# facebookresearch/AudioDec

Measured on NVIDIA H100. Metric: 48 kHz audio samples/s, encode+quantize+lookup+decode (% HBM roofline in `roofline`), higher is better.
Workload: dtype f32

## Files before the change

audiodec_b200/csrc/wg_conv.cuh:

```cuda
#pragma once
#include <cuda_bf16.h>
#include <cuda_fp16.h>

#include "kernels.cuh"

namespace adec {

constexpr int TC_TT = 128;
constexpr int TC_CP = 32;
constexpr int TC_MIDP = 128;
constexpr float F16_LO_SCALE = 2048.f;
enum { PREC_BF16 = 1, PREC_TF32 = 2, PREC_F16 = 3 };

__device__ __forceinline__ void fence_async_smem() { asm volatile("fence.proxy.async.shared::cta;" ::: "memory"); }
__device__ __forceinline__ float tf32_rna(float x) {
    uint32_t r;
    asm("cvt.rna.tf32.f32 %0, %1;" : "=r"(r) : "f"(x));
    return __uint_as_float(r);
}

__device__ __forceinline__ uint64_t wg_desc(uint32_t saddr, uint32_t lbo_bytes) {
    return (uint64_t)((saddr & 0x3FFFF) >> 4) | ((uint64_t)((lbo_bytes >> 4) & 0x3FFF) << 16) | ((uint64_t)(128 >> 4) << 32);
}
__device__ __forceinline__ void wg_fence() { asm volatile("wgmma.fence.sync.aligned;" ::: "memory"); }
__device__ __forceinline__ void wg_commit() { asm volatile("wgmma.commit_group.sync.aligned;" ::: "memory"); }
__device__ __forceinline__ void wg_wait0() { asm volatile("wgmma.wait_group.sync.aligned 0;" ::: "memory"); }
template <int N>
__device__ __forceinline__ void wg_fence_regs(float (&d)[N]) {
#pragma unroll
    for (int i = 0; i < N; ++i) asm volatile("" : "+f"(d[i])::"memory");
}

template <int N, int PREC> struct Wgmma;
#define ADEC_WG_N32(PREC, TYPE, TAIL)                                                                                              \
    template <> struct Wgmma<32, PREC> {                                                                                           \
        __device__ __forceinline__ static void mma(float (&d)[16], uint64_t da, uint64_t db, uint32_t acc) {                     \
            asm volatile("{\n .reg .pred p;\n setp.ne.b32 p, %18, 0;\n wgmma.mma_async.sync.aligned.m64n32" TYPE                \
                         " {%0,%1,%2,%3,%4,%5,%6,%7,%8,%9,%10,%11,%12,%13,%14,%15}, %16, %17, p, 1, 1" TAIL ";\n}"                  \
                         : "+f"(d[0]), "+f"(d[1]), "+f"(d[2]), "+f"(d[3]), "+f"(d[4]), "+f"(d[5]), "+f"(d[6]), "+f"(d[7]),          \
                           "+f"(d[8]), "+f"(d[9]), "+f"(d[10]), "+f"(d[11]), "+f"(d[12]), "+f"(d[13]), "+f"(d[14]), "+f"(d[15])     \
                         : "l"(da), "l"(db), "r"(acc));                                                                            \
        }                                                                                                                          \
    };
#define ADEC_WG_N64(PREC, TYPE, TAIL)                                                                                              \
    template <> struct Wgmma<64, PREC> {                                                                                           \
        __device__ __forceinline__ static void mma(float (&d)[32], uint64_t da, uint64_t db, uint32_t acc) {                     \
            asm volatile("{\n .reg .pred p;\n setp.ne.b32 p, %34, 0;\n wgmma.mma_async.sync.aligned.m64n64" TYPE                \
                         " {%0,%1,%2,%3,%4,%5,%6,%7,%8,%9,%10,%11,%12,%13,%14,%15,%16,%17,%18,%19,%20,%21,%22,%23,%24,%25,%26,%27," \
                         "%28,%29,%30,%31}, %32, %33, p, 1, 1" TAIL ";\n}"                                                          \
                         : "+f"(d[0]), "+f"(d[1]), "+f"(d[2]), "+f"(d[3]), "+f"(d[4]), "+f"(d[5]), "+f"(d[6]), "+f"(d[7]),          \
                           "+f"(d[8]), "+f"(d[9]), "+f"(d[10]), "+f"(d[11]), "+f"(d[12]), "+f"(d[13]), "+f"(d[14]), "+f"(d[15]),    \
                           "+f"(d[16]), "+f"(d[17]), "+f"(d[18]), "+f"(d[19]), "+f"(d[20]), "+f"(d[21]), "+f"(d[22]), "+f"(d[23]),  \
                           "+f"(d[24]), "+f"(d[25]), "+f"(d[26]), "+f"(d[27]), "+f"(d[28]), "+f"(d[29]), "+f"(d[30]), "+f"(d[31])   \
                         : "l"(da), "l"(db), "r"(acc));                                                                            \
        }                                                                                                                          \
    };
ADEC_WG_N32(PREC_F16, "k16.f32.f16.f16", ", 0, 0")
ADEC_WG_N32(PREC_BF16, "k16.f32.bf16.bf16", ", 0, 0")
ADEC_WG_N32(PREC_TF32, "k8.f32.tf32.tf32", "")
ADEC_WG_N64(PREC_F16, "k16.f32.f16.f16", ", 0, 0")
ADEC_WG_N64(PREC_BF16, "k16.f32.bf16.bf16", ", 0, 0")
ADEC_WG_N64(PREC_TF32, "k8.f32.tf32.tf32", "")
#undef ADEC_WG_N32
#undef ADEC_WG_N64

template <int NT, int PREC> struct WgCfg {
    static constexpr int EB = PREC == PREC_TF32 ? 4 : 2;
    static constexpr int KBB = TC_CP * EB / 16;
    static constexpr int NPR = PREC == PREC_F16 ? 3 : PREC == PREC_TF32 ? 2 : 1;
    static constexpr int NPL = PREC == PREC_BF16 ? 1 : 2;
    static constexpr int TPG = PREC == PREC_TF32 ? 1 : 2;
    static constexpr int TAP_BYTES = NPR * KBB * NT * 16;
    static constexpr int STAGE_BYTES = TPG * TAP_BYTES;
    static constexpr int MID_BYTES = NPL * (NT * EB / 16) * TC_MIDP * 16;
    __host__ __device__ static constexpr int stages(bool fuse) { return PREC == PREC_TF32 && NT == 128 && fuse ? 1 : NT == 128 ? 2 : 3; }
    static constexpr int PW = NT < 64 ? NT : 64;
    static constexpr int NPROD = 96;
    static constexpr int THREADS = 256 + NPROD + 32;
    __host__ __device__ static constexpr int win_pitch(int wrows) { return ((wrows + 1) & ~3) + 2; }
    __host__ __device__ static constexpr int win_bytes(int wrows) { return NPL * KBB * win_pitch(wrows) * 16; }
    static int n_wbuf(int wrows, bool fuse) {
        const long long avail = 227 * 1024 - 512 - (long long)stages(fuse) * STAGE_BYTES - (fuse ? (long long)MID_BYTES : 0);
        const long long n = avail / win_bytes(wrows);
        return (int)(n > 4 ? 4 : n);
    }
    static size_t smem_bytes(int wrows, bool fuse) {
        return 512 + (size_t)stages(fuse) * STAGE_BYTES + (size_t)n_wbuf(wrows, fuse) * win_bytes(wrows) + (fuse ? (size_t)MID_BYTES : 0);
    }
};

template <int ACT>
__device__ __forceinline__ float4 apply_act_t(float4 v, float slope) {
    if (ACT == ACT_ELU) { v.x = act_elu(v.x); v.y = act_elu(v.y); v.z = act_elu(v.z); v.w = act_elu(v.w); }
    if (ACT == ACT_LRELU) { v.x = act_lrelu(v.x, slope); v.y = act_lrelu(v.y, slope); v.z = act_lrelu(v.z, slope); v.w = act_lrelu(v.w, slope); }
    return v;
}

__device__ __forceinline__ uint32_t h2_bits(__half2 h) { return *reinterpret_cast<const uint32_t*>(&h); }
__device__ __forceinline__ uint32_t b2_bits(__nv_bfloat162 h) { return *reinterpret_cast<const uint32_t*>(&h); }
template <int PREC>
__device__ __forceinline__ void split2(float x, float y, uint2& hi, uint2& lo) {
    if (PREC == PREC_F16) {
        const __half2 h = __floats2half2_rn(x, y);
        const float2 f = __half22float2(h);
        hi.x = h2_bits(h);
        lo.x = h2_bits(__floats2half2_rn((x - f.x) * F16_LO_SCALE, (y - f.y) * F16_LO_SCALE));
    } else if (PREC == PREC_TF32) {
        const float hx = tf32_rna(x), hy = tf32_rna(y);
        hi = make_uint2(__float_as_uint(hx), __float_as_uint(hy));
        lo = make_uint2(__float_as_uint(x - hx), __float_as_uint(y - hy));
    } else {
        hi.x = b2_bits(__floats2bfloat162_rn(x, y));
    }
}
template <int PREC>
__device__ __forceinline__ void split_store(unsigned char* hi, unsigned char* lo, size_t bstride, const float4 u, const float4 v) {
    uint2 h0, l0, h1, l1, h2, l2, h3, l3;
    split2<PREC>(u.x, u.y, h0, l0); split2<PREC>(u.z, u.w, h1, l1);
    split2<PREC>(v.x, v.y, h2, l2); split2<PREC>(v.z, v.w, h3, l3);
    if (PREC == PREC_TF32) {
        *reinterpret_cast<uint4*>(hi) = make_uint4(h0.x, h0.y, h1.x, h1.y);
        *reinterpret_cast<uint4*>(hi + bstride) = make_uint4(h2.x, h2.y, h3.x, h3.y);
        *reinterpret_cast<uint4*>(lo) = make_uint4(l0.x, l0.y, l1.x, l1.y);
        *reinterpret_cast<uint4*>(lo + bstride) = make_uint4(l2.x, l2.y, l3.x, l3.y);
    } else {
        *reinterpret_cast<uint4*>(hi) = make_uint4(h0.x, h1.x, h2.x, h3.x);
        if (PREC == PREC_F16) *reinterpret_cast<uint4*>(lo) = make_uint4(l0.x, l1.x, l2.x, l3.x);
    }
}

struct TileIter {
    int tile, xt, y, b, sx, sy, sb, nx, ny;
    __device__ __forceinline__ TileIter(int first, int step, int n_x, int n_y) {
        nx = n_x; ny = n_y; tile = first;
        xt = first % n_x;
        const int q = first / n_x;
        y = q % n_y; b = q / n_y;
        sx = step % n_x;
        const int sq = step / n_x;
        sy = sq % n_y; sb = sq / n_y;
    }
    __device__ __forceinline__ void next(int step) {
        tile += step;
        xt += sx;
        const int cx = xt >= nx ? 1 : 0;
        xt -= cx ? nx : 0;
        y += sy + cx;
        const int cy = y >= ny ? 1 : 0;
        y -= cy ? ny : 0;
        b += sb + cy;
    }
};

__device__ __forceinline__ float4 norm4(float4 x, const float* mean, const float* scale) {
    const float4 mu = *reinterpret_cast<const float4*>(mean);
    const float4 sc = *reinterpret_cast<const float4*>(scale);
    x.x = __fdiv_rn(x.x - mu.x, sc.x); x.y = __fdiv_rn(x.y - mu.y, sc.y);
    x.z = __fdiv_rn(x.z - mu.z, sc.z); x.w = __fdiv_rn(x.w - mu.w, sc.w);
    return x;
}

template <int NT, int PREC>
__device__ __forceinline__ void wg_group(float (&d)[WgCfg<NT, PREC>::PW / 2], uint32_t a_hi, uint32_t a_lo, uint32_t lbo, uint32_t tap_step,
                                         int ntaps, uint32_t bw) {
    using Cfg = WgCfg<NT, PREC>;
    constexpr int NKS = Cfg::KBB / 2, TPG = Cfg::TPG;
    constexpr uint32_t B_LBO = NT * 16u, B_KS = 2u * NT * 16u, B_T = Cfg::TAP_BYTES, B_PL = Cfg::KBB * NT * 16u;
    constexpr uint32_t PL_SMALL = PREC == PREC_F16 ? 2u : 0u;
    uint32_t acc = 0u;
    wg_fence_regs(d);
    wg_fence();
    if (PREC != PREC_BF16) {
#pragma unroll
        for (int t = 0; t < TPG; ++t)
#pragma unroll
            for (int ks = 0; ks < NKS; ++ks)
                if (t < ntaps) {
                    Wgmma<Cfg::PW, PREC>::mma(d, wg_desc(a_lo + t * tap_step + ks * 2u * lbo, lbo), wg_desc(bw + t * B_T + PL_SMALL * B_PL + ks * B_KS, B_LBO), acc);
                    acc = 1u;
                }
#pragma unroll
        for (int t = 0; t < TPG; ++t)
#pragma unroll
            for (int ks = 0; ks < NKS; ++ks)
                if (t < ntaps) Wgmma<Cfg::PW, PREC>::mma(d, wg_desc(a_hi + t * tap_step + ks * 2u * lbo, lbo), wg_desc(bw + t * B_T + B_PL + ks * B_KS, B_LBO), 1u);
    }
#pragma unroll
    for (int t = 0; t < TPG; ++t)
#pragma unroll
        for (int ks = 0; ks < NKS; ++ks)
            if (t < ntaps) {
                Wgmma<Cfg::PW, PREC>::mma(d, wg_desc(a_hi + t * tap_step + ks * 2u * lbo, lbo), wg_desc(bw + t * B_T + ks * B_KS, B_LBO), acc);
                acc = 1u;
            }
    wg_commit();
    wg_wait0();
    wg_fence_regs(d);
}

template <int NT, bool FUSE, int PRE, int PREC>
__global__ void __launch_bounds__(WgCfg<NT, PREC>::THREADS, 1) wg_conv_kernel(const ConvArgs a, int n_xtiles, int n_ytiles, int n_tiles) {
    using Cfg = WgCfg<NT, PREC>;
    constexpr int S = Cfg::stages(FUSE), CP = TC_CP, TT = TC_TT, KBB = Cfg::KBB, EB = Cfg::EB, TPG = Cfg::TPG, PW = Cfg::PW;
    constexpr int NPROD = Cfg::NPROD, WWARP = (256 + NPROD) / 32;
    constexpr int STAGE_BYTES = Cfg::STAGE_BYTES, TAP_BYTES = Cfg::TAP_BYTES;
    constexpr int NH = NT / PW;
    constexpr int NACC = NT / 2;
    constexpr int MBLK = NT * EB / 16;

    extern __shared__ __align__(128) unsigned char smem_raw[];
    uint64_t* b_full = reinterpret_cast<uint64_t*>(smem_raw);
    uint64_t* b_empty = b_full + S;
    uint64_t* w_full = b_empty + S;
    uint64_t* w_empty = w_full + 4;
    unsigned char* bst = smem_raw + 512;
    const int wrows = TT + (a.Ktaps - 1) * a.dil;
    const int wrp = Cfg::win_pitch(wrows);
    const int win_b = Cfg::win_bytes(wrows);
    unsigned char* wbuf0 = bst + S * STAGE_BYTES;
    unsigned char* mbuf = wbuf0 + (size_t)a.n_wbuf * win_b;

    const int tid = threadIdx.x, lane = tid & 31;
    const int warp = __shfl_sync(0xffffffffu, tid >> 5, 0);
    unsigned long long kt0 = 0;
    long long kc0 = 0;
    if (a.dbg && blockIdx.x == 0 && tid == 0) { asm volatile("mov.u64 %0, %%globaltimer;" : "=l"(kt0)); kc0 = clock64(); }
    if (tid == 0) {
        for (int s = 0; s < S; ++s) { mbar_init(&b_full[s], 1); mbar_init(&b_empty[s], 2); }
        for (int i = 0; i < 4; ++i) { mbar_init(&w_full[i], NPROD); mbar_init(&w_empty[i], 2); }
        mbar_fence_init();
    }
    __syncthreads();
    asm volatile("griddepcontrol.launch_dependents;" ::: "memory");
    if (warp != WWARP) asm volatile("griddepcontrol.wait;" ::: "memory");

    if (warp == WWARP) {
        if (lane == 0) {
            int c = 0;
            auto stream = [&](const unsigned char* base, int pieces, int taps) {
                for (int p = 0; p < pieces; ++p)
                    for (int t0 = 0; t0 < taps; t0 += TPG, ++c) {
                        const int s = c % S, it = c / S;
                        const uint32_t bytes = (uint32_t)(taps - t0 >= TPG ? TPG : taps - t0) * TAP_BYTES;
                        if (it > 0) mbar_wait(&b_empty[s], (it - 1) & 1, 100);
                        mbar_arrive_expect_tx(&b_full[s], bytes);
                        bulk_g2s(bst + s * STAGE_BYTES, base + ((long long)p * taps + t0) * TAP_BYTES, bytes, &b_full[s]);
                    }
            };
            const unsigned char* w1 = reinterpret_cast<const unsigned char*>(a.w);
            const unsigned char* w2 = reinterpret_cast<const unsigned char*>(a.w2);
            for (TileIter it(blockIdx.x, gridDim.x, n_xtiles, n_ytiles); it.tile < n_tiles; it.next(gridDim.x)) {
                stream(w1 + (long long)it.y * a.w_tile_floats * 4, a.n_pieces, a.Ktaps);
                if (FUSE) stream(w2, NT / CP, 1);
            }
        }
    } else if (warp >= 8) {
        const int pt = tid - 256;
        int wb = 0, wround = 0;
        constexpr int RPP = NPROD / 4;
        constexpr int UNR = 6;
        constexpr int UNR_E = 6;
        const int c8 = pt & 3, m0 = pt >> 2;
        const size_t bstride = (size_t)wrp * 16;
        const bool halves = a.RG > 1 && a.Cin < 8;
        for (TileIter it(blockIdx.x, gridDim.x, n_xtiles, n_ytiles); it.tile < n_tiles; it.next(gridDim.x)) {
            const int xt = it.xt, y = it.y, b = it.b;
            int g = 0, co_tile = y;
            if (a.n_co_tiles != n_ytiles) { g = y / a.n_co_tiles; co_tile = y - g * a.n_co_tiles; }
            const int j0 = xt * TT;
            const float* xg = a.x + (long long)b * a.x_bs + g * a.x_goff;
            const float* sg = a.st_in + (long long)b * a.P * a.st_ld + g * a.st_goff;
            for (int p = 0; p < a.n_pieces; ++p) {
                const int buf = wb;
                const uint32_t wpar = (uint32_t)(wround - 1) & 1u;
                bool waited = wround == 0;
                if (++wb == a.n_wbuf) { wb = 0; ++wround; }
                unsigned char* hi = wbuf0 + (size_t)buf * win_b + (size_t)c8 * (KBB / 4) * bstride;
                unsigned char* lo = hi + (size_t)KBB * bstride;
                const int q = p * CP + c8 * 8;
                int r = 0, ci = q;
                if (a.RG > 1) { r = q >> a.lgCin; ci = q & (a.Cin - 1); }
                const long long i_first = (long long)j0 * a.RG + r;
                const long long i_last = (long long)(j0 + wrows - 1) * a.RG + r;
                if (i_first >= a.P && i_last - a.P < a.T && PRE != ACT_NORM && !halves && !a.stack_L) {
                    const float* xp = xg + ci + (i_first - a.P + (long long)m0 * a.RG) * a.ldx;
                    const long long xstep = (long long)RPP * a.RG * a.ldx;
                    for (int mb = m0; mb < wrows; mb += RPP * UNR, xp += xstep * UNR) {
                        float4 u[UNR], v[UNR];
#pragma unroll
                        for (int k = 0; k < UNR; ++k)
                            if (mb + k * RPP < wrows) {
                                u[k] = __ldg(reinterpret_cast<const float4*>(xp + k * xstep));
                                v[k] = __ldg(reinterpret_cast<const float4*>(xp + k * xstep) + 1);
                            }
                        if (!waited) { mbar_wait(&w_empty[buf], wpar, 500); waited = true; }
#pragma unroll
                        for (int k = 0; k < UNR; ++k) {
                            const int m = mb + k * RPP;
                            if (m < wrows) split_store<PREC>(hi + m * 16, lo + m * 16, bstride, apply_act_t<PRE>(u[k], a.slope), apply_act_t<PRE>(v[k], a.slope));
                        }
                    }
                } else {
                    int ci2 = ci + 4;
                    for (int mb = m0; mb < wrows; mb += RPP * UNR_E) {
                        float4 u[UNR_E], v[UNR_E];
                        unsigned act = 0u;
#pragma unroll
                        for (int k = 0; k < UNR_E; ++k) {
                            const int m = mb + k * RPP;
                            u[k] = v[k] = make_float4(0.f, 0.f, 0.f, 0.f);
                            if (m < wrows) {
                                int ml = j0 + m;
                                const float* xs = xg;
                                const float* ss = sg;
                                bool live = true;
                                if (a.stack_L) {
                                    const int sm = ml / a.stack_L;
                                    ml -= sm * a.stack_L;
                                    live = sm < a.n_streams;
                                    xs = xg + (long long)sm * a.x_bs;
                                    ss = sg + (long long)sm * a.P * a.st_ld;
                                }
#pragma unroll
                                for (int hf = 0; hf < 2; ++hf) {
                                    int rr = r, cc = ci + 4 * hf;
                                    if (halves) { rr = (q + 4 * hf) >> a.lgCin; cc = (q + 4 * hf) & (a.Cin - 1); if (hf) ci2 = cc; }
                                    const long long i = (long long)ml * a.RG + rr;
                                    long long ti = i - a.P;
                                    if (a.hist_rep && ti < 0) ti = 0;
                                    float4 w4 = make_float4(0.f, 0.f, 0.f, 0.f);
                                    if (live) {
                                        if (ti < 0) w4 = __ldg(reinterpret_cast<const float4*>(ss + i * a.st_ld + cc));
                                        else if (ti < a.T) { w4 = __ldg(reinterpret_cast<const float4*>(xs + ti * a.ldx + cc)); act |= 1u << (2 * k + hf); }
                                    }
                                    if (hf) v[k] = w4; else u[k] = w4;
                                }
                            }
                        }
                        if (!waited) { mbar_wait(&w_empty[buf], wpar, 500); waited = true; }
#pragma unroll
                        for (int k = 0; k < UNR_E; ++k) {
                            const int m = mb + k * RPP;
                            if (m < wrows) {
                                float4 x0 = u[k], x1 = v[k];
                                if ((act >> (2 * k)) & 1u) x0 = PRE == ACT_NORM ? norm4(x0, a.mean + ci, a.scale + ci) : apply_act_t<PRE>(x0, a.slope);
                                if ((act >> (2 * k)) & 2u) x1 = PRE == ACT_NORM ? norm4(x1, a.mean + ci2, a.scale + ci2) : apply_act_t<PRE>(x1, a.slope);
                                split_store<PREC>(hi + m * 16, lo + m * 16, bstride, x0, x1);
                            }
                        }
                    }
                }
                fence_async_smem();
                mbar_arrive(&w_full[buf]);
            }
            if (co_tile == 0 && g < a.st_groups && a.P > 0) {
                int s_lo = b, s_hi = b - 1;
                if (a.stack_L) {
                    s_lo = (j0 - (a.Tout - 1) + a.stack_L - 1) / a.stack_L;
                    if (j0 < a.Tout - 1) s_lo = 0;
                    s_hi = (j0 + TT - 1 - (a.Tout - 1)) / a.stack_L;
                    if (j0 + TT - 1 < a.Tout - 1) s_hi = -1;
                    if (s_hi > a.n_streams - 1) s_hi = a.n_streams - 1;
                } else if (xt == (a.Tout - 1) / TT) {
                    s_hi = b;
                }
                for (int sm = s_lo; sm <= s_hi; ++sm) {
                    const float* xs = a.x + (long long)sm * a.x_bs + g * a.x_goff;
                    const float* ss = a.st_in + (long long)sm * a.P * a.st_ld + g * a.st_goff;
                    float* so = a.st_out + (long long)sm * a.P * a.st_ld + g * a.st_goff;
                    const int nvec = a.P * (a.Cin / 4);
                    for (int idx = pt; idx < nvec; idx += NPROD) {
                        const int r = idx / (a.Cin / 4);
                        const int cc = (idx - r * (a.Cin / 4)) * 4;
                        const long long i = (long long)a.T + r;
                        float4 w4;
                        if (i < a.P) {
                            w4 = *reinterpret_cast<const float4*>(ss + i * a.st_ld + cc);
                        } else {
                            w4 = __ldg(reinterpret_cast<const float4*>(xs + (i - a.P) * a.ldx + cc));
                            if (PRE == ACT_NORM) w4 = norm4(w4, a.mean + cc, a.scale + cc);
                            else w4 = apply_act_t<PRE>(w4, a.slope);
                        }
                        *reinterpret_cast<float4*>(so + (long long)r * a.st_ld + cc) = w4;
                    }
                }
            }
        }
    } else {
        const int wg = warp >> 2;
        const int wrow = 64 * wg + 16 * (warp & 3) + (lane >> 2), col2 = 2 * (lane & 3);
        const uint32_t row0_off = (uint32_t)(64 * wg) * 16u;
        const uint32_t wbuf0_u = smem_u32(wbuf0), mbuf_u = smem_u32(mbuf), bst_u = smem_u32(bst);
        const uint32_t lbo1 = (uint32_t)wrp * 16u, lbo2 = (uint32_t)TC_MIDP * 16u;
        const uint32_t tap_step = (uint32_t)a.dil * 16u;
        float racc[NACC];
        float part[PW / 2];
#pragma unroll
        for (int i = 0; i < PW / 2; ++i) part[i] = 0.f;
        int c = 0, wb = 0, wround = 0;
        float vmax = 0.f;
        auto group = [&](uint32_t a_hi, uint32_t a_lo, uint32_t lbo, uint32_t row_off, int ntaps) {
            const int s = c % S;
            mbar_wait(&b_full[s], (c / S) & 1, 300);
            const uint32_t bw = bst_u + (uint32_t)s * STAGE_BYTES;
#pragma unroll
            for (int h = 0; h < NH; ++h) {
                wg_group<NT, PREC>(part, a_hi + row_off, a_lo + row_off, lbo, tap_step, ntaps, bw + (uint32_t)h * PW * 16u);
#pragma unroll
                for (int i = 0; i < PW / 2; ++i) racc[h * (PW / 2) + i] = __fadd_rn(racc[h * (PW / 2) + i], part[i]);
            }
            if (threadIdx.x % 128 == 0) mbar_arrive(&b_empty[s]);
            ++c;
        };
        for (TileIter it(blockIdx.x, gridDim.x, n_xtiles, n_ytiles); it.tile < n_tiles; it.next(gridDim.x)) {
            const int xt = it.xt, y = it.y, b = it.b;
            int g = 0, co_tile = y;
            if (a.n_co_tiles != n_ytiles) { g = y / a.n_co_tiles; co_tile = y - g * a.n_co_tiles; }
            const int j0 = xt * TT;
#pragma unroll
            for (int i = 0; i < NACC; ++i) racc[i] = 0.f;
            for (int p = 0; p < a.n_pieces; ++p) {
                const int buf = wb;
                mbar_wait(&w_full[buf], wround & 1, 200);
                if (++wb == a.n_wbuf) { wb = 0; ++wround; }
                const uint32_t a_hi = wbuf0_u + (uint32_t)buf * (uint32_t)win_b;
                for (int t0 = 0; t0 < a.Ktaps; t0 += TPG)
                    group(a_hi, a_hi + (uint32_t)KBB * lbo1, lbo1, row0_off + (uint32_t)t0 * tap_step, a.Ktaps - t0 >= TPG ? TPG : a.Ktaps - t0);
                if (threadIdx.x % 128 == 0) mbar_arrive(&w_empty[buf]);
            }
            if (FUSE) {
#pragma unroll
                for (int i = 0; i < NACC; i += 4) {
                    const float4 m4 = apply_act_t<PRE>(make_float4(racc[i] * a.w_scale, racc[i + 1] * a.w_scale, racc[i + 2] * a.w_scale, racc[i + 3] * a.w_scale), a.slope);
                    racc[i] = m4.x; racc[i + 1] = m4.y; racc[i + 2] = m4.z; racc[i + 3] = m4.w;
                    vmax = fmaxf(vmax, fmaxf(fmaxf(fabsf(m4.x), fabsf(m4.y)), fmaxf(fabsf(m4.z), fabsf(m4.w))));
                }
#pragma unroll
                for (int i = 0; i < NACC; i += 2) {
                    const int h = i / (PW / 2), fi = i % (PW / 2);
                    const int co = h * PW + 8 * (fi >> 2) + col2, row = wrow + 8 * ((fi >> 1) & 1);
                    const int blk = co * EB / 16, off = (co * EB) & 15;
                    unsigned char* hp = mbuf + ((size_t)blk * TC_MIDP + row) * 16 + off;
                    uint2 hi, lo;
                    split2<PREC>(racc[i], racc[i + 1], hi, lo);
                    if (PREC == PREC_TF32) {
                        *reinterpret_cast<uint2*>(hp) = hi;
                        *reinterpret_cast<uint2*>(hp + (size_t)MBLK * TC_MIDP * 16) = lo;
                    } else {
                        *reinterpret_cast<uint32_t*>(hp) = hi.x;
                        if (PREC == PREC_F16) *reinterpret_cast<uint32_t*>(hp + (size_t)MBLK * TC_MIDP * 16) = lo.x;
                    }
                }
                fence_async_smem();
                named_bar_sync(1 + wg, 128);
#pragma unroll
                for (int i = 0; i < NACC; ++i) racc[i] = 0.f;
                for (int p = 0; p < NT / CP; ++p) {
                    const uint32_t m_hi = mbuf_u + (uint32_t)(p * KBB) * lbo2;
                    group(m_hi, m_hi + (uint32_t)MBLK * lbo2, lbo2, row0_off, 1);
                }
            }
            const float oscale = FUSE ? a.w2_scale : a.w_scale;
#pragma unroll
            for (int hr = 0; hr < 2; ++hr) {
                int bo = b, t = j0 + wrow + 8 * hr;
                if (a.stack_L) { bo = t / a.stack_L; t -= bo * a.stack_L; }
                if (!(t < a.Tout && bo < a.n_streams)) continue;
#pragma unroll
                for (int i = 2 * hr; i < NACC; i += 4) {
                    const int h = i / (PW / 2), fi = i % (PW / 2);
                    const int co_l = co_tile * NT + h * PW + 8 * (fi >> 2) + col2;
                    if (co_l >= a.Cout_g) continue;
                    float v0 = racc[i] * oscale, v1 = racc[i + 1] * oscale;
                    if (a.bias) {
                        const float2 b2 = __ldg(reinterpret_cast<const float2*>(a.bias + g * a.Cout_g + co_l));
                        v0 += b2.x; v1 += b2.y;
                    }
                    if (a.res) {
                        const float2 r2 = __ldg(reinterpret_cast<const float2*>(a.res + (long long)bo * a.res_bs + (long long)t * a.ldr + g * a.r_goff + co_l));
                        v0 = r2.x + v0; v1 = r2.y + v1;
                    }
                    vmax = fmaxf(vmax, fmaxf(fabsf(v0), fabsf(v1)));
                    if (a.out_nct) {
                        float* yp = a.y + (long long)bo * a.y_bs + (long long)(g * a.y_goff + co_l) * a.Tout + t;
                        yp[0] = v0;
                        yp[a.Tout] = v1;
                    } else {
                        *reinterpret_cast<float2*>(a.y + (long long)bo * a.y_bs + (long long)t * a.ldy + g * a.y_goff + co_l) = make_float2(v0, v1);
                    }
                }
            }
        }
        if (PREC == PREC_F16 && a.err && !(vmax < 60000.f)) atomicOr(a.err, 2);
    }
    if (a.dbg && blockIdx.x == 0 && tid == 0) {
        unsigned long long kt1;
        asm volatile("mov.u64 %0, %%globaltimer;" : "=l"(kt1));
        a.dbg[0] = kt0; a.dbg[1] = kt1; a.dbg[2] = (unsigned long long)(clock64() - kc0);
    }
}

__device__ float g_probe_sink;
template <int NT, int PREC>
__global__ void __launch_bounds__(256) mma_probe_kernel(int n_groups, int a_pitch_rows) {
    using Cfg = WgCfg<NT, PREC>;
    constexpr int PW = Cfg::PW, KSTEPS = 8;
    extern __shared__ __align__(128) unsigned char smem[];
    const int a_bytes = KSTEPS * 2 * a_pitch_rows * 16;
    for (int i = threadIdx.x; i < a_bytes / 16 + KSTEPS * 2 * NT; i += 256) reinterpret_cast<uint4*>(smem)[i] = make_uint4(0u, 0u, 0u, 0u);
    fence_async_smem();
    __syncthreads();
    const int wg = threadIdx.x >> 7;
    const uint32_t a_u = smem_u32(smem) + (uint32_t)(64 * wg) * 16u, b_u = smem_u32(smem + a_bytes);
    const uint32_t a_lbo = (uint32_t)a_pitch_rows * 16u, b_lbo = (uint32_t)NT * 16u;
    float d[PW / 2];
#pragma unroll
    for (int i = 0; i < PW / 2; ++i) d[i] = 0.f;
    float sink = 0.f;
    for (int g = 0; g < n_groups; ++g) {
#pragma unroll 1
        for (int h = 0; h < NT / PW; ++h) {
            wg_fence_regs(d);
            wg_fence();
#pragma unroll
            for (int k = 0; k < 12; ++k) {
                const uint32_t ks = (uint32_t)((g * 12 + k) % KSTEPS);
                Wgmma<PW, PREC>::mma(d, wg_desc(a_u + ks * 2u * a_lbo, a_lbo), wg_desc(b_u + ks * 2u * b_lbo + (uint32_t)h * PW * 16u, b_lbo), k ? 1u : 0u);
            }
            wg_commit();
            wg_wait0();
            wg_fence_regs(d);
            sink += d[0];
        }
    }
    if (sink != 0.f) g_probe_sink = sink;
}

}
```

Measured before the change: 115.6 million.

## Double-buffer wgmma accumulators to overlap tensor-core groups with partial-sum adds

Replaces the issue-then-wait-0 pattern in the wgmma conv consumer with a software pipeline: two accumulator register sets alternate so one group's wgmma runs while the previous group's partials are added into racc, using wait_group 1. Stage and window buffer releases are deferred until the owning group retires. The tap count becomes a template parameter, which removes runtime predicates. For the NT=32 fused path it also prefetches bias and residual loads before the final wait. This adds register pressure and more complex barrier bookkeeping, and n_wbuf now returns 0 when too few window buffers fit.

New measurement: 116.5 million, median of 6. No clear change (+0.7%).

```diff
diff --git a/audiodec_b200/csrc/wg_conv.cuh b/audiodec_b200/csrc/wg_conv.cuh
--- a/audiodec_b200/csrc/wg_conv.cuh
+++ b/audiodec_b200/csrc/wg_conv.cuh
@@ -1,6 +1,8 @@
 #pragma once
 #include <cuda_bf16.h>
 #include <cuda_fp16.h>
+
+#include <type_traits>
 
 #include "kernels.cuh"
 
@@ -24,7 +26,6 @@
 }
 __device__ __forceinline__ void wg_fence() { asm volatile("wgmma.fence.sync.aligned;" ::: "memory"); }
 __device__ __forceinline__ void wg_commit() { asm volatile("wgmma.commit_group.sync.aligned;" ::: "memory"); }
-__device__ __forceinline__ void wg_wait0() { asm volatile("wgmma.wait_group.sync.aligned 0;" ::: "memory"); }
 template <int N>
 __device__ __forceinline__ void wg_fence_regs(float (&d)[N]) {
 #pragma unroll
@@ -82,6 +83,7 @@
     static int n_wbuf(int wrows, bool fuse) {
         const long long avail = 227 * 1024 - 512 - (long long)stages(fuse) * STAGE_BYTES - (fuse ? (long long)MID_BYTES : 0);
         const long long n = avail / win_bytes(wrows);
+        if (n < (stages(fuse) > 1 ? 2 : 1)) return 0;
         return (int)(n > 4 ? 4 : n);
     }
     static size_t smem_bytes(int wrows, bool fuse) {
@@ -160,42 +162,34 @@
     return x;
 }
 
-template <int NT, int PREC>
+template <int N> __device__ __forceinline__ void wg_wait() { asm volatile("wgmma.wait_group.sync.aligned %0;" ::"n"(N) : "memory"); }
+
+template <int NT, int PREC, int NTAPS>
 __device__ __forceinline__ void wg_group(float (&d)[WgCfg<NT, PREC>::PW / 2], uint32_t a_hi, uint32_t a_lo, uint32_t lbo, uint32_t tap_step,
-                                         int ntaps, uint32_t bw) {
+                                         uint32_t bw) {
     using Cfg = WgCfg<NT, PREC>;
-    constexpr int NKS = Cfg::KBB / 2, TPG = Cfg::TPG;
+    constexpr int NKS = Cfg::KBB / 2;
     constexpr uint32_t B_LBO = NT * 16u, B_KS = 2u * NT * 16u, B_T = Cfg::TAP_BYTES, B_PL = Cfg::KBB * NT * 16u;
     constexpr uint32_t PL_SMALL = PREC == PREC_F16 ? 2u : 0u;
-    uint32_t acc = 0u;
-    wg_fence_regs(d);
-    wg_fence();
     if (PREC != PREC_BF16) {
 #pragma unroll
-        for (int t = 0; t < TPG; ++t)
+        for (int t = 0; t < NTAPS; ++t)
 #pragma unroll
             for (int ks = 0; ks < NKS; ++ks)
-                if (t < ntaps) {
-                    Wgmma<Cfg::PW, PREC>::mma(d, wg_desc(a_lo + t * tap_step + ks * 2u * lbo, lbo), wg_desc(bw + t * B_T + PL_SMALL * B_PL + ks * B_KS, B_LBO), acc);
-                    acc = 1u;
-                }
-#pragma unroll
-        for (int t = 0; t < TPG; ++t)
+                Wgmma<Cfg::PW, PREC>::mma(d, wg_desc(a_lo + t * tap_step + ks * 2u * lbo, lbo), wg_desc(bw + t * B_T + PL_SMALL * B_PL + ks * B_KS, B_LBO),
+                                          (t | ks) ? 1u : 0u);
+#pragma unroll
+        for (int t = 0; t < NTAPS; ++t)
 #pragma unroll
             for (int ks = 0; ks < NKS; ++ks)
-                if (t < ntaps) Wgmma<Cfg::PW, PREC>::mma(d, wg_desc(a_hi + t * tap_step + ks * 2u * lbo, lbo), wg_desc(bw + t * B_T + B_PL + ks * B_KS, B_LBO), 1u);
-    }
-#pragma unroll
-    for (int t = 0; t < TPG; ++t)
+                Wgmma<Cfg::PW, PREC>::mma(d, wg_desc(a_hi + t * tap_step + ks * 2u * lbo, lbo), wg_desc(bw + t * B_T + B_PL + ks * B_KS, B_LBO), 1u);
+    }
+#pragma unroll
+    for (int t = 0; t < NTAPS; ++t)
 #pragma unroll
         for (int ks = 0; ks < NKS; ++ks)
-            if (t < ntaps) {
-                Wgmma<Cfg::PW, PREC>::mma(d, wg_desc(a_hi + t * tap_step + ks * 2u * lbo, lbo), wg_desc(bw + t * B_T + ks * B_KS, B_LBO), acc);
-                acc = 1u;
-            }
-    wg_commit();
-    wg_wait0();
-    wg_fence_regs(d);
+            Wgmma<Cfg::PW, PREC>::mma(d, wg_desc(a_hi + t * tap_step + ks * 2u * lbo, lbo), wg_desc(bw + t * B_T + ks * B_KS, B_LBO),
+                                      (PREC != PREC_BF16 || (t | ks)) ? 1u : 0u);
 }
 
 template <int NT, bool FUSE, int PRE, int PREC>
@@ -393,24 +387,89 @@
         const uint32_t wbuf0_u = smem_u32(wbuf0), mbuf_u = smem_u32(mbuf), bst_u = smem_u32(bst);
         const uint32_t lbo1 = (uint32_t)wrp * 16u, lbo2 = (uint32_t)TC_MIDP * 16u;
         const uint32_t tap_step = (uint32_t)a.dil * 16u;
+        const bool leader = threadIdx.x % 128 == 0;
         float racc[NACC];
-        float part[PW / 2];
-#pragma unroll
-        for (int i = 0; i < PW / 2; ++i) part[i] = 0.f;
+        float pa[PW / 2], pb[PW / 2];
+#pragma unroll
+        for (int i = 0; i < PW / 2; ++i) pa[i] = pb[i] = 0.f;
         int c = 0, wb = 0, wround = 0;
         float vmax = 0.f;
-        auto group = [&](uint32_t a_hi, uint32_t a_lo, uint32_t lbo, uint32_t row_off, int ntaps) {
+        constexpr bool PIPE = S > 1 && NT != 64;
+        using I0 = std::integral_constant<int, 0>;
+        using I1 = std::integral_constant<int, 1>;
+        struct GOps { uint32_t a_hi, a_lo, lbo; bool full; int win; };
+        int rel_s[2] = {-1, -1}, rel_w[2] = {-1, -1};
+        auto add = [&](const float (&d)[PW / 2], int h) {
+#pragma unroll
+            for (int i = 0; i < PW / 2; ++i) racc[h * (PW / 2) + i] = __fadd_rn(racc[h * (PW / 2) + i], d[i]);
+        };
+        auto issue = [&](auto xc, const GOps& o) {
+            constexpr int X = decltype(xc)::value, H = NH == 2 ? X : 0;
             const int s = c % S;
-            mbar_wait(&b_full[s], (c / S) & 1, 300);
-            const uint32_t bw = bst_u + (uint32_t)s * STAGE_BYTES;
-#pragma unroll
-            for (int h = 0; h < NH; ++h) {
-                wg_group<NT, PREC>(part, a_hi + row_off, a_lo + row_off, lbo, tap_step, ntaps, bw + (uint32_t)h * PW * 16u);
-#pragma unroll
-                for (int i = 0; i < PW / 2; ++i) racc[h * (PW / 2) + i] = __fadd_rn(racc[h * (PW / 2) + i], part[i]);
-            }
-            if (threadIdx.x % 128 == 0) mbar_arrive(&b_empty[s]);
-            ++c;
+            if (H == 0) mbar_wait(&b_full[s], (c / S) & 1, 300);
+            const uint32_t bw = bst_u + (uint32_t)s * STAGE_BYTES + (uint32_t)H * PW * 16u;
+            wg_fence_regs(pa);
+            wg_fence_regs(pb);
+            wg_fence();
+            if (o.full) wg_group<NT, PREC, TPG>(X ? pb : pa, o.a_hi, o.a_lo, o.lbo, tap_step, bw);
+            else wg_group<NT, PREC, 1>(X ? pb : pa, o.a_hi, o.a_lo, o.lbo, tap_step, bw);
+            wg_commit();
+            wg_fence_regs(pa);
+            wg_fence_regs(pb);
+            rel_s[X] = H == NH - 1 ? s : -1;
+            rel_w[X] = H == NH - 1 ? o.win : -1;
+            if (H == NH - 1) ++c;
+        };
+        auto retire = [&](auto xc, auto nc) {
+            constexpr int X = decltype(xc)::value, H = NH == 2 ? X : 0;
+            wg_wait<decltype(nc)::value>();
+            wg_fence_regs(pa);
+            wg_fence_regs(pb);
+            add(X ? pb : pa, H);
+            if (leader && rel_s[X] >= 0) mbar_arrive(&b_empty[rel_s[X]]);
+            if (leader && rel_w[X] >= 0) mbar_arrive(&w_empty[rel_w[X]]);
+        };
+        auto phase = [&](int G, auto next) -> int {
+            if (!PIPE) {
+                for (int gi = 0; gi < G; ++gi) {
+                    const GOps o = next();
+                    issue(I0(), o);
+                    retire(I0(), I0());
+                    if (NH == 2) { issue(I1(), o); retire(I1(), I0()); }
+                }
+                return 0;
+            }
+            if (NH == 2) {
+                GOps o = next();
+                issue(I0(), o);
+                issue(I1(), o);
+                retire(I0(), I1());
+                for (int gi = 1; gi < G; ++gi) {
+                    o = next();
+                    issue(I0(), o);
+                    retire(I1(), I1());
+                    issue(I1(), o);
+                    retire(I0(), I1());
+                }
+                return 1;
+            }
+            issue(I0(), next());
+            int gi = 1;
+            for (; gi + 1 < G; gi += 2) {
+                issue(I1(), next());
+                retire(I0(), I1());
+                issue(I0(), next());
+                retire(I1(), I1());
+            }
+            if (gi == G) return 0;
+            issue(I1(), next());
+            retire(I0(), I1());
+            return 1;
+        };
+        auto finish = [&](int last) {
+            if (!PIPE) return;
+            if (last) retire(I1(), I0());
+            else retire(I0(), I0());
         };
         for (TileIter it(blockIdx.x, gridDim.x, n_xtiles, n_ytiles); it.tile < n_tiles; it.next(gridDim.x)) {
             const int xt = it.xt, y = it.y, b = it.b;
@@ -419,16 +478,22 @@
             const int j0 = xt * TT;
 #pragma unroll
             for (int i = 0; i < NACC; ++i) racc[i] = 0.f;
-            for (int p = 0; p < a.n_pieces; ++p) {
-                const int buf = wb;
-                mbar_wait(&w_full[buf], wround & 1, 200);
-                if (++wb == a.n_wbuf) { wb = 0; ++wround; }
-                const uint32_t a_hi = wbuf0_u + (uint32_t)buf * (uint32_t)win_b;
-                for (int t0 = 0; t0 < a.Ktaps; t0 += TPG)
-                    group(a_hi, a_hi + (uint32_t)KBB * lbo1, lbo1, row0_off + (uint32_t)t0 * tap_step, a.Ktaps - t0 >= TPG ? TPG : a.Ktaps - t0);
-                if (threadIdx.x % 128 == 0) mbar_arrive(&w_empty[buf]);
-            }
+            int t0 = 0, buf = 0;
+            const int last = phase(a.n_pieces * ((a.Ktaps + TPG - 1) / TPG), [&]() {
+                if (t0 == 0) {
+                    buf = wb;
+                    mbar_wait(&w_full[buf], wround & 1, 200);
+                    if (++wb == a.n_wbuf) { wb = 0; ++wround; }
+                }
+                const uint32_t a_hi = wbuf0_u + (uint32_t)buf * (uint32_t)win_b + row0_off + (uint32_t)t0 * tap_step;
+                const GOps o{a_hi, a_hi + (uint32_t)KBB * lbo1, lbo1, a.Ktaps - t0 >= TPG, t0 + TPG >= a.Ktaps ? buf : -1};
+                t0 += TPG;
+                if (t0 >= a.Ktaps) t0 = 0;
+                return o;
+            });
+            int last2 = last;
             if (FUSE) {
+                finish(last);
 #pragma unroll
                 for (int i = 0; i < NACC; i += 4) {
                     const float4 m4 = apply_act_t<PRE>(make_float4(racc[i] * a.w_scale, racc[i + 1] * a.w_scale, racc[i + 2] * a.w_scale, racc[i + 3] * a.w_scale), a.slope);
@@ -455,11 +520,31 @@
                 named_bar_sync(1 + wg, 128);
 #pragma unroll
                 for (int i = 0; i < NACC; ++i) racc[i] = 0.f;
-                for (int p = 0; p < NT / CP; ++p) {
-                    const uint32_t m_hi = mbuf_u + (uint32_t)(p * KBB) * lbo2;
-                    group(m_hi, m_hi + (uint32_t)MBLK * lbo2, lbo2, row0_off, 1);
-                }
-            }
+                int p = 0;
+                last2 = phase(NT / CP, [&]() {
+                    const uint32_t m_hi = mbuf_u + (uint32_t)(p++ * KBB) * lbo2 + row0_off;
+                    return GOps{m_hi, m_hi + (uint32_t)MBLK * lbo2, lbo2, TPG == 1, -1};
+                });
+            }
+            constexpr bool PF = NT == 32 && FUSE;
+            float2 rpf[PF ? NACC / 2 : 1], bpf[PF ? NACC / 4 : 1];
+            if (PF) {
+#pragma unroll
+                for (int hr = 0; hr < 2; ++hr) {
+                    int bo = b, t = j0 + wrow + 8 * hr;
+                    if (a.stack_L) { bo = t / a.stack_L; t -= bo * a.stack_L; }
+                    const bool row_ok = t < a.Tout && bo < a.n_streams;
+#pragma unroll
+                    for (int i = 2 * hr; i < NACC; i += 4) {
+                        const int co_l = co_tile * NT + 8 * (i >> 2) + col2;
+                        if (co_l >= a.Cout_g) continue;
+                        if (hr == 0 && a.bias) bpf[i >> 2] = __ldg(reinterpret_cast<const float2*>(a.bias + g * a.Cout_g + co_l));
+                        if (row_ok && a.res)
+                            rpf[i >> 1] = __ldg(reinterpret_cast<const float2*>(a.res + (long long)bo * a.res_bs + (long long)t * a.ldr + g * a.r_goff + co_l));
+                    }
+                }
+            }
+            finish(last2);
             const float oscale = FUSE ? a.w2_scale : a.w_scale;
 #pragma unroll
             for (int hr = 0; hr < 2; ++hr) {
@@ -473,11 +558,12 @@
                     if (co_l >= a.Cout_g) continue;
                     float v0 = racc[i] * oscale, v1 = racc[i + 1] * oscale;
                     if (a.bias) {
-                        const float2 b2 = __ldg(reinterpret_cast<const float2*>(a.bias + g * a.Cout_g + co_l));
+                        const float2 b2 = PF ? bpf[i >> 2] : __ldg(reinterpret_cast<const float2*>(a.bias + g * a.Cout_g + co_l));
                         v0 += b2.x; v1 += b2.y;
                     }
                     if (a.res) {
-                        const float2 r2 = __ldg(reinterpret_cast<const float2*>(a.res + (long long)bo * a.res_bs + (long long)t * a.ldr + g * a.r_goff + co_l));
+                        const float2 r2 = PF ? rpf[i >> 1]
+                                             : __ldg(reinterpret_cast<const float2*>(a.res + (long long)bo * a.res_bs + (long long)t * a.ldr + g * a.r_goff + co_l));
                         v0 = r2.x + v0; v1 = r2.y + v1;
                     }
                     vmax = fmaxf(vmax, fmaxf(fabsf(v0), fabsf(v1)));
@@ -528,7 +614,7 @@
                 Wgmma<PW, PREC>::mma(d, wg_desc(a_u + ks * 2u * a_lbo, a_lbo), wg_desc(b_u + ks * 2u * b_lbo + (uint32_t)h * PW * 16u, b_lbo), k ? 1u : 0u);
             }
             wg_commit();
-            wg_wait0();
+            wg_wait<0>();
             wg_fence_regs(d);
             sink += d[0];
         }
```
